# mmSir/SpatioTemporalEntropyModel

Hardware: AMD Instinct MI355X
Metric: frames/s (higher is better)
Workload: dtype f32; 1 GPU; configs[1]: SpatioTemporalPriorModel_Res(256,192) training step on mbt2018(192,192) latents, 16 septuplets x 7 frames x 256x256 per GPU, EMLoss, clip 1.0 + Adam 1e-4 / aux Adam 1e-3; per_gpu_batch=16, global_batch=16, parallelism=dp1, stream_priorities=latents=0,side=-1,compute=-1, stream_cu_masks=latents=block:160, plan_selectors=library defaults

## Files before the change

### include/stem_hip.h

```cpp
#ifndef STEM_HIP_H
#define STEM_HIP_H

#include <stddef.h>
#include <stdint.h>

#ifdef __cplusplus
extern "C" {
#endif

const char *stem_last_error(void);
int stem_abi_version(void);

void *stem_tape_create(void);
void stem_tape_destroy(void *tape);
int stem_tape_length(void *tape);
int stem_tape_add_call(void *tape, void *fn, int nargs, const unsigned char *kinds, const long long *ivals, const double *fvals,
                       const long long *ideltas);
int stem_tape_add_wait(void *tape, void *waiting_stream, void *signalling_stream);
int stem_tape_add_event(void *tape, void *event, void *stream, int wait);
int stem_tape_replay(void *tape, int lo, int hi, long long n);
int stem_tape_set_iarg(void *tape, int entry, int arg, long long value);
int stem_tape_set_farg(void *tape, int entry, int arg, double pattern);
int stem_tape_entry_recordable(void *fn);
int stem_copy_d2d(void *dst, const void *src, size_t nbytes, void *stream);
int stem_zero_bytes(void *dst, size_t nbytes, void *stream);
int stem_stream_flag_create(void **flag);
int stem_stream_flag_destroy(void *flag);
int stem_stream_flag_wait_ge(void *flag, unsigned value, void *stream);
int stem_stream_flag_write(void *flag, unsigned value, void *stream);
int stem_tuning_set(const char *name, int value);
int stem_tuning_get(const char *name);

enum {
    STEM_PACK_CONV_FWD = 0,
    STEM_PACK_CONV_DGRAD = 1,
    STEM_PACK_DECONV_FWD = 2,
    STEM_PACK_DECONV_DGRAD = 3,
    STEM_PACK_CONV_FWD_C4 = 4
};
int stem_pack_weight(const float *w, float *wp, int K, int C, int R, int S, int role, int masked, void *stream);
size_t stem_packed_weight_elems(int K, int C, int R, int S, int role);
enum { STEM_UNPACK_DECONV = 1, STEM_UNPACK_ACCUMULATE = 2 };
int stem_unpack_wgrad(const float *dwp, float *dw, int K, int C, int R, int S, int splits, int flags, void *stream);

typedef struct {
    const float *w;
    float *wp;
    int K, C, R, S, role, masked;
} stem_pack_desc;
typedef struct {
    const float *dwp;
    float *dw;
    int K, C, R, S, splits;
    int flags;
} stem_unpack_desc;
int stem_pack_weights_multi(const stem_pack_desc *descs, int n, void *stream);
int stem_unpack_wgrads_multi(const stem_unpack_desc *descs, int n, void *stream);
typedef struct {
    const float *part;
    float *db;
    int K, parts, accumulate, reserved;
} stem_bias_final_desc;
int stem_bias_grad_final_multi(const stem_bias_final_desc *descs, int n, void *stream);

enum { STEM_ACT_NONE = 0, STEM_ACT_LRELU = 1 };
// ... 287 lines not shown
```

### spatiotemporalentropymodel_amd/config.py

```python
from __future__ import annotations

import contextlib
import dataclasses
import os
from dataclasses import dataclass


@dataclass
class StemRuntimeConfig:
    analysis_f16x3: bool = True
    first_layer_f16x3: bool = True
    engine_f16x3: bool = True
    engine_strided_f16x3: bool = True
    engine_transposed_f16x3: bool = True
    engine_ctx_f16x3: bool = True
    engine_wgrad_f16x3: bool = True
    engine_records: bool = True
    layers_f16x3: bool = True
    layers_f16x3_maxpix: int = 1 << 30
    layers_wide_minpix: int = 32768
    trainer_overwrite_grads: bool = True
    adam_block_max: bool = True
    engine_overlap: bool = True
    engine_split_pack: bool = True
    engine_pack_pair: bool = True
    engine_branch: bool = True
    engine_tail_ordered: bool = True
    stream_prio: str = ""
    stream_cumask: str = ""
    dp_threaded: int = 3
    dp_min_bytes: int = 8 << 20
    dist_backend: str = ""
    dist_single: bool = False
    pin_ranks: bool = True
    ar_persistent: bool = True
    ar_stepwise: bool = False
    ar_force_batch: bool = False
    ar_concurrent: bool = True
    ar_no_batch: bool = False


_ENV = {
    "analysis_f16x3": "STEM_F16X3", "first_layer_f16x3": "STEM_C4GDN_F16X3", "engine_f16x3": "STEM_ENGINE_F16X3",
    "engine_strided_f16x3": "STEM_ENGINE_STRIDED_F16X3", "engine_transposed_f16x3": "STEM_ENGINE_TRANSPOSED_F16X3", "engine_ctx_f16x3": "STEM_ENGINE_CTX_F16X3",
    "engine_wgrad_f16x3": "STEM_ENGINE_WGRAD_F16X3", "engine_records": "STEM_ENGINE_RECORDS", "layers_f16x3": "STEM_LAYERS_F16X3",
    "layers_f16x3_maxpix": "STEM_LAYERS_F16X3_MAXPIX", "layers_wide_minpix": "STEM_LAYERS_WIDE_MINPIX",
    "adam_block_max": "STEM_ADAM_BLOCK_MAX", "trainer_overwrite_grads": "STEM_TRAINER_OVERWRITE_GRADS", "engine_overlap": "STEM_ENGINE_OVERLAP",
    "engine_split_pack": "STEM_ENGINE_SPLIT_PACK", "engine_pack_pair": "STEM_ENGINE_PACK_PAIR", "engine_branch": "STEM_ENGINE_BRANCH",
    "engine_tail_ordered": "STEM_ENGINE_TAIL_ORDERED",
    "stream_prio": "STEM_STREAM_PRIO", "stream_cumask": "STEM_STREAM_CUMASK", "dp_min_bytes": "STEM_DP_MIN_BYTES", "dp_threaded": "STEM_DP_THREADED",
    "dist_backend": "STEM_DIST_BACKEND", "dist_single": "STEM_DIST_SINGLE", "pin_ranks": "STEM_PIN_RANKS",
    "ar_persistent": "STEM_AR_PERSISTENT", "ar_stepwise": "STEM_AR_STEPWISE",
    "ar_force_batch": "STEM_AR_FORCE_BATCH", "ar_concurrent": "STEM_AR_CONCURRENT", "ar_no_batch": "STEM_AR_NO_BATCH",
}


def _parse(kind, text):
    if kind is bool:
        return text.strip() not in ("", "0", "false", "False", "no", "off")
    if kind is int:
        return int(text)
    return text


def from_env(environ=None) -> StemRuntimeConfig:
    environ = os.environ if environ is None else environ
    cfg = StemRuntimeConfig()
    for f in dataclasses.fields(cfg):
        name = _ENV[f.name]
        if name in environ:
            setattr(cfg, f.name, _parse(type(f.default), environ[name]))
    return cfg
# ... 48 lines not shown
```

### spatiotemporalentropymodel_amd/csrc/pack.hip

```cpp
#include <stdarg.h>

#include "stem_common.h"

static thread_local char g_err[512] = "";
void stem_set_error(const char *fmt, ...)
{
    va_list ap;
    va_start(ap, fmt);
    vsnprintf(g_err, sizeof(g_err), fmt, ap);
    va_end(ap);
}
STEM_EXPORT const char *stem_last_error(void) { return g_err; }
STEM_EXPORT int stem_abi_version(void) { return 5; }

static int g_tuning[STEM_TUNE_COUNT] = {0};
static const char *const kTuningNames[STEM_TUNE_COUNT] = {"fx3_tile", "fx3_split", "wg3_split", "arp_workers", "fx3_depth", "fx3_gen_tile", "fx3_mfma", "fx3_gen_mfma", "fx3_gen_img", "fx3_img_w", "wg3_row", "wg3_minch", "tconv_cps", "arp_giveup_at", "unpack_mb", "igemm_cfg", "igemm_fuse_cfg", "igemm_split", "wgrad_cfg"};
static int g_ran[STEM_RAN_COUNT] = {0};
static const char *const kRanNames[STEM_RAN_COUNT] = {"igemm_ran_cfg", "igemm_ran_split", "wgrad_ran_cfg", "fx3_ran_form", "fx3_ran_split", "fx3_ran_mfma", "wg3_ran_form", "wg3_ran_taps", "wg3_ran_split", "fx3_col_ran_tile", "fx3_col_ran_depth", "fx3_col_ran_mfma", "tconv_ran_tile", "tconv_ran_cps", "tconv_ran_split0", "tconv_ran_split1", "tconv_ran_split2", "tconv_ran_split3"};
void stem_ran_note(int id, int value) { g_ran[id] = value; }
int stem_tuning(int id) { return g_tuning[id]; }
STEM_EXPORT int stem_tuning_set(const char *name, int value)
{
    STEM_CHECK_ARG(name && value >= 0, "stem_tuning_set: null name or negative value");
    for (int i = 0; i < STEM_RAN_COUNT; ++i)
        STEM_CHECK_ARG(strcmp(name, kRanNames[i]), "stem_tuning_set: %s is get-only (the plan of the most recent launch)", name);
// ... 71 lines not shown
    const int n = d.Bd * d.T;
    for (int k = threadIdx.x; k < n; k += 256) {
        const int b = k / d.T, t = k - b * d.T;
        float v = d.w[a * d.sa + b * d.sb + t];
        if (d.masked & 3) {
            const int r = t / d.S, s = t - r * d.S;
            if (r > d.R / 2 || (r == d.R / 2 && s >= d.S / 2 + ((d.masked >> 2) & 1))) {
                v = 0.f;
                if ((d.masked & 3) == 2) d.w[a * d.sa + b * d.sb + t] = 0.f;
            }
        }
        tile[k] = v;
    }
    __syncthreads();
    for (int k = threadIdx.x; k < n; k += 256) {
        const int t = k / d.Bd, b = k - t * d.Bd;
        d.out[((size_t)t * d.A + a) * d.Bd + b] = tile[b * d.T + t];
    }
}

struct UnpackD {
    const float *dwp;
    float *dw;
    int A, Bd, T, splits, block0, accumulate, mb;
};
struct UnpackTable {
    UnpackD d[MAXD];
    int n;
};
constexpr int UNPACK_MB = 64, UNPACK_MB_MAX = 192;
__global__ __launch_bounds__(256) void unpack_multi_kernel(const UnpackTable tb)
{
    extern __shared__ float tile[];
    int i = 0;
    while (i + 1 < tb.n && (int)blockIdx.x >= tb.d[i + 1].block0) ++i;
    const UnpackD d = tb.d[i];
    const int mb = d.mb;
    const int chunks = (d.Bd + mb - 1) / mb;
    const int blk = blockIdx.x - d.block0;
    const int a = blk / chunks, b0 = (blk - a * chunks) * mb;
    const int nb = d.Bd - b0 < mb ? d.Bd - b0 : mb;
    const int n = nb * d.T;
    const size_t slab = (size_t)d.T * d.A * d.Bd;
    const bool vec = nb == mb && (d.Bd & 3) == 0 && ((reinterpret_cast<uintptr_t>(d.dwp) | reinterpret_cast<uintptr_t>(d.dw)) & 15) == 0 &&
                     ((size_t)d.Bd * d.T) % 4 == 0 && (slab & 3) == 0;
    if (vec) {
        const int q = mb / 4, n4 = d.T * q;
        for (int k = threadIdx.x; k < n4; k += 256) {
            const int t = k / q, b4 = k - t * q;
            const f32x4 *src = reinterpret_cast<const f32x4 *>(d.dwp + ((size_t)t * d.A + a) * d.Bd + b0) + b4;
            f32x4 v0 = {0.f, 0.f, 0.f, 0.f}, v1 = {0.f, 0.f, 0.f, 0.f};
            int sp = 0;
            for (; sp + 3 < d.splits; sp += 4) {
                const f32x4 x0 = src[(size_t)sp * (slab / 4)], x1 = src[(size_t)(sp + 1) * (slab / 4)];
                const f32x4 x2 = src[(size_t)(sp + 2) * (slab / 4)], x3 = src[(size_t)(sp + 3) * (slab / 4)];
                v0 += x0; v1 += x1; v0 += x2; v1 += x3;
            }
            for (; sp + 1 < d.splits; sp += 2) {
                const f32x4 x0 = src[(size_t)sp * (slab / 4)], x1 = src[(size_t)(sp + 1) * (slab / 4)];
                v0 += x0; v1 += x1;
            }
            if (sp < d.splits) v0 += src[(size_t)sp * (slab / 4)];
            const f32x4 v = v0 + v1;
#pragma unroll
            for (int j = 0; j < 4; ++j) tile[(b4 * 4 + j) * (d.T + 1) + t] = v[j];
        }
        __syncthreads();
        float *dst = d.dw + ((size_t)a * d.Bd + b0) * d.T;
        for (int k4 = threadIdx.x; k4 < n / 4; k4 += 256) {
            f32x4 v;
#pragma unroll
            for (int j = 0; j < 4; ++j) {
                const int k = 4 * k4 + j, b = k / d.T, t = k - b * d.T;
                v[j] = tile[b * (d.T + 1) + t];
            }
            f32x4 *o = reinterpret_cast<f32x4 *>(dst) + k4;
            *o = d.accumulate ? *o + v : v;
        }
        return;
    }
    for (int k = threadIdx.x; k < n; k += 256) {
        const int t = k / nb, b = k - t * nb;
        const float *src = d.dwp + ((size_t)t * d.A + a) * d.Bd + b0 + b;
        float v0 = 0.f, v1 = 0.f;
        int s = 0;
        for (; s + 1 < d.splits; s += 2) {
            v0 += src[s * slab];
            v1 += src[(s + 1) * slab];
        }
        if (s < d.splits) v0 += src[s * slab];
        tile[b * (d.T + 1) + t] = v0 + v1;
    }
    __syncthreads();
    float *dst = d.dw + ((size_t)a * d.Bd + b0) * d.T;
    for (int k = threadIdx.x; k < n; k += 256) {
        const int b = k / d.T, t = k - b * d.T;
        const float v = tile[b * (d.T + 1) + t];
        dst[k] = d.accumulate ? dst[k] + v : v;
    }
}

__global__ void pack_c4_kernel(const float *w, float *out, int K, int C, int T)
{
    const int i = blockIdx.x * blockDim.x + threadIdx.x;
    if (i >= K * 128) return;
    const int k = i >> 7, r = i & 127, t = r >> 2, c = r & 3;
    out[i] = (t < T && c < C) ? w[((size_t)k * C + c) * T + t] : 0.f;
}

constexpr int UNPACK_BT = 32;
__global__ __launch_bounds__(256) void unpack_kernel(const float *dwp, float *dw, int A, int Bd, int T, int splits, int accumulate)
{
    extern __shared__ float tile[];
    const int a = blockIdx.x, b0 = blockIdx.y * UNPACK_BT;
    const int nb = Bd - b0 < UNPACK_BT ? Bd - b0 : UNPACK_BT;
    const int n = nb * T;
    const size_t slab = (size_t)T * A * Bd;
    for (int i = threadIdx.x; i < n; i += 256) {
        const int t = i / nb, b = i - t * nb;
        const float *src = dwp + ((size_t)t * A + a) * Bd + b0 + b;
        float v0 = 0.f, v1 = 0.f;
        int s = 0;
// ... 146 lines not shown
            const stem_pack_desc &q = descs[base + i];
            PackD &d = tb.d[i];
            const int T = q.R * q.S;
            STEM_CHECK_ARG(q.w && q.wp && T >= 1 && T <= 25, "stem_pack_weights_multi: bad descriptor %d", base + i);
            STEM_CHECK_ARG(role_geometry(q.role, q.K, q.C, T, &d.A, &d.Bd, &d.sa, &d.sb) == 0,
                           "stem_pack_weights_multi: role %d not supported in the multi-tensor path", q.role);
            d.w = const_cast<float *>(q.w);
            d.out = q.wp;
            d.T = T; d.R = q.R; d.S = q.S; d.masked = q.masked;
            d.block0 = blocks;
            blocks += d.A;
            const size_t need = (size_t)d.Bd * T * sizeof(float);
            if (need > lds) lds = need;
        }
        STEM_CHECK_ARG(lds <= 160 * 1024, "stem_pack_weights_multi: slab of %zu B exceeds LDS", lds);
        if (lds > 64 * 1024)
            (void)hipFuncSetAttribute((const void *)pack_multi_kernel, hipFuncAttributeMaxDynamicSharedMemorySize, (int)lds);
        if (blocks) hipLaunchKernelGGL(pack_multi_kernel, dim3(blocks), dim3(256), lds, st, tb);
        STEM_LAUNCH_CHECK("pack_multi");
    }
    return 0;
}

STEM_EXPORT int stem_unpack_wgrads_multi(const stem_unpack_desc *descs, int n, void *stream)
{
    STEM_CHECK_ARG(descs && n >= 0, "stem_unpack_wgrads_multi: bad arguments");
    hipStream_t st = (hipStream_t)stream;
    for (int base = 0; base < n; base += MAXD) {
        UnpackTable tb;
        tb.n = n - base < MAXD ? n - base : MAXD;
        int blocks = 0;
        size_t lds = 0;
        for (int i = 0; i < tb.n; ++i) {
            const stem_unpack_desc &q = descs[base + i];
            UnpackD &d = tb.d[i];
            STEM_CHECK_ARG(q.dwp && q.dw && q.splits >= 1, "stem_unpack_wgrads_multi: bad descriptor %d", base + i);
            d.dwp = q.dwp; d.dw = q.dw;
            d.T = q.R * q.S;
            const int deconv = q.flags & STEM_UNPACK_DECONV;
            d.accumulate = (q.flags & STEM_UNPACK_ACCUMULATE) ? 1 : 0;
            d.A = deconv ? q.C : q.K;
            d.Bd = deconv ? q.K : q.C;
            d.splits = q.splits;
            d.block0 = blocks;
            const int forced_mb = stem_tuning(STEM_TUNE_UNPACK_MB);
            d.mb = UNPACK_MB;
            if (forced_mb) {
                d.mb = forced_mb;
            } else {
                for (int mb = UNPACK_MB_MAX; mb > UNPACK_MB; mb -= 32)
                    if (d.Bd % mb == 0 && (long)d.A * (d.Bd / mb) >= 512) {
                        d.mb = mb;
                        break;
                    }
            }
            blocks += d.A * cdiv(d.Bd, d.mb);
            const size_t need = (size_t)d.mb * (d.T + 1) * sizeof(float);
            if (need > lds) lds = need;
        }
        if (blocks) hipLaunchKernelGGL(unpack_multi_kernel, dim3(blocks), dim3(256), lds, st, tb);
        STEM_LAUNCH_CHECK("unpack_multi");
    }
    return 0;
}

STEM_EXPORT int stem_unpack_wgrad(const float *dwp, float *dw, int K, int C, int R, int S, int splits, int flags,
                                  void *stream)
{
    STEM_CHECK_ARG(dwp && dw && splits >= 1, "stem_unpack_wgrad: bad arguments");
    const int T = R * S;
    const int deconv = flags & STEM_UNPACK_DECONV;
    const int A = deconv ? C : K, Bd = deconv ? K : C;
    const size_t lds = (size_t)UNPACK_BT * (T + 1) * sizeof(float);
    STEM_CHECK_ARG(lds <= 64 * 1024, "stem_unpack_wgrad: %d taps exceed the staging tile", T);
    hipLaunchKernelGGL(unpack_kernel, dim3(A, cdiv(Bd, UNPACK_BT)), dim3(256), lds, (hipStream_t)stream, dwp, dw, A, Bd, T, splits,
                       (flags & STEM_UNPACK_ACCUMULATE) ? 1 : 0);
    STEM_LAUNCH_CHECK("unpack");
    return 0;
}

STEM_EXPORT int stem_nchw_to_nhwc(const float *x, float *y, int ldy, int B, int C, int H, int W, void *stream)
{
    STEM_CHECK_ARG(x && y && ldy >= C, "stem_nchw_to_nhwc: bad arguments");
    const int HW = H * W;
// ... 36 lines not shown
```

### spatiotemporalentropymodel_amd/engine.py

```python
from __future__ import annotations

import collections

import torch

from . import _lib
from . import config as _config
from . import functional as F
from . import layers as _layers

class _Switch:

    def __init__(self, field):
        self.field = field

    def __get__(self, obj, owner=None):
        return getattr(_config._RUNTIME or _config.runtime(), self.field)


class _Act:
    __slots__ = ("x", "p", "rec")

    def __init__(self, x, p=None, rec=None):
        self.x, self.p, self.rec = x, p, rec
# ... 130 lines not shown
        return _Act(F.deconv2d_fwd(a.x, self.wp_fwd, m.bias, self.K, self.R, self.R, self.stride, self.pad, self.opad, act, out=out))

    def fwd(self, x, act=F.ACT_NONE, out=None):
        return self.forward(_Act(x), act, out=out).x

    def input_grad(self, dy, xact=None, planes=False, x_shape=None):
        if self.tail_event is not None:
            self.eng._wait_tail(self)
        face = self.faces[1]
        epi = F.GEN_EPI_DACT if xact is not None else F.GEN_EPI_BIAS
        if face.kind == "gen":
            return _Act(*F.conv2d_f16x3_gen(dy.planes(), self.wp6_dgrad, None, self.C, self.R, self.R, self.stride, self.pad,
                                            epi=epi, z=xact, want_planes=planes))
        if face.kind == "phases":
            return _Act(*F.tconv2d_f16x3(dy.planes(), self.wp6_dgrad, None, self.C, self.R, epi=epi, z=xact, want_planes=planes,
                                         fine_hw=tuple(xact.shape[2:]) if xact is not None else None))
        x_shape = xact.shape if xact is not None else x_shape
        if self.kind == "conv":
            return _Act(F.conv2d_dgrad(dy.x, self.wp_dgrad, x_shape, self.K, self.R, self.R, self.stride, self.pad, xact=xact))
        return _Act(F.deconv2d_dgrad(dy.x, self.wp_dgrad, x_shape, self.K, self.R, self.R, self.stride, self.pad, self.opad, xact=xact))

    def reads_dy_planes(self, x):
        return self.faces[1].kind != "f32" if self.faces[1] is not None else (self.wg3 and x.p is not None)

    def weight_grad(self, x, dy):
        at_hand = (x.p is not None) + (dy.p is not None)
        if self.fx3t:
            fn, args = self._wgrad_t, ((x.planes(), dy.planes()) if self.kind == "conv" else (dy.planes(), x.planes())) + (dy.x,)
        elif self.wg3 and at_hand >= (2 if self.need_dgrad else 1):
            fn, args = self._wgrad3, (x.planes(record=False), dy.planes(record=False), dy.x)
        else:
            fn, args = self._wgrad, (x.x, dy.x)
        side = self.eng.side_stream(dy.x.device, self.lane)
        if side is None:
            return fn(*args)
        F.stream_wait(side, F.cur_stream(dy.x.device))
        with F.on_stream(side):
            fn(*args)
        for t in args:
            (t.data if isinstance(t, F.F16Planes) else t).record_stream(side)

    def _wgrad_t(self, fine_p, coarse_p, dy):
        conv = self.kind == "conv"
        Kk = self.K if conv else self.C
        key = ("fp16t",) + tuple(fine_p.shape)
        if key not in self._slabs:
# ... 334 lines not shown

    def _drop_tail(self):
        self.join_tail()
        self._tail_last = None
        self._tail_waited.clear()
        for l in self.layers:
            l.tail_event = None

    def unpack_all(self):
        for lane in sorted({l.lane for l in self.layers}):
            self._group_ready([l for l in self.layers if l.lane == lane], [])

    grad_ready_hook = None

    def _group_ready(self, layers, extra_params):
        dev = layers[0].mod.weight.device
        side = self.side_stream(dev, layers[0].lane)
        if side is None:
            return self._group_ready_on_stream(layers, extra_params)
        F.stream_wait(side, F.cur_stream(dev))
        with F.on_stream(side):
            self._group_ready_on_stream(layers, extra_params)

    def _group_ready_on_stream(self, layers, extra_params):
        bdescs = [l.pending_bias for l in layers if getattr(l, "pending_bias", None) is not None]
        for l in layers:
            l.pending_bias = None
        if bdescs:
            F.bias_grad_final_multi(bdescs)
        descs = [l.unpack_desc() for l in layers if l.pending is not None]
        if descs:
            arr = (_lib.UnpackDesc * len(descs))(*descs)
            F.unpack_wgrads_multi(arr)
        if self.grad_ready_hook is not None:
            params = [p for l in layers for p in (l.mod.weight, l.mod.bias) if p is not None] + list(extra_params)
            if params:
                hook = self.grad_ready_hook
                F.tape_py(lambda: hook(params))

    def join_side_stream(self):
        for st in self._side.values():
            F.stream_wait(F.cur_stream(st.device), st)

    def _wait_fwd32_packs(self):
        if self._fwd32_pack_event is not None:
            F.event_wait(F.cur_stream(), self._fwd32_pack_event)

    def _wait_dgrad_packs(self):
        if self._dgrad_pack_event is not None:
            F.event_wait(F.cur_stream(), self._dgrad_pack_event)
            self._dgrad_pack_event = None

    def forward(self, y_cur, y_cond, training: bool, rate_coef=None):
        self.ensure_packed()
        self._checked = True
        try:
# ... 89 lines not shown
            else:
                z_hat, lik_z = F.eb_forward(z, pack, medians=eb._medians_vec())
            acts["z_hat"], acts["hd0"], acts["hd2"], _ = self._chain_forward(self.HD, _Act(z_hat, rec=rec.get("z_hat")), out=epm_in[:, o_hp:o_hp + P], planes=ep)
        if not fused:
            target = F.sub(yc, yd) if self.residual else (yc if F.nhwc_ld(yc) == Cin else F.copy_channels(yc, F.empty_nhwc(B, Cin, H, W, dev)))
        if self.has_spm:
            if not fused:
                t_hat = F.add(target, gc._noise_like(target)) if training else F.round_(target)
                acts["t_hat"] = _Act(t_hat)
            if ctx_split_done is not None:
                F.event_wait(F.cur_stream(dev), ctx_split_done)
            self.CTX.forward(acts["t_hat"], out=epm_in[:, o_ctx:o_ctx + P])
        if bs is not None:
            F.stream_wait(main, bs)
        acts["epm_in"], acts["e0"], acts["e2"], gp = self._chain_forward(self.EPM, _Act(epm_in), planes=ep)
        gp = gp.x
        scales, means = gp[:, :Cin], gp[:, Cin:]
        if fused:
            dgp = F.empty_nhwc(B, 2 * Cin, H, W, dev)
            gc_out, lik_y, k["dlik_y"], part_y, k["qg"] = F.gc_forward_train(
                target, scales, means, rate_coef[0], scale_bound=gc._scale_bound, lik_bound=gc._lik_bound,
                backward=(dgp[:, :Cin], dgp[:, Cin:]), record=self.EPM[0].fx3 and self.use_records, **gc._noise_slot(target))
            k["dgp"] = dgp
            k["loss3"] = F.em_loss_finalize(part_y, part_z, rate_coef[1])
            if not self.has_spm:
                y_hat = gc_out
        else:
            noise = gc._noise_like(target) if training else None
            gc_out, lik_y = F.gc_forward(target, scales, means, noise=noise, scale_bound=gc._scale_bound, lik_bound=gc._lik_bound)
            if self.has_spm:
                y_hat = F.add(t_hat, yd if F.nhwc_ld(yd) == Cin else F.copy_channels(yd, F.empty_nhwc(B, Cin, H, W, dev))) if self.residual else t_hat
            else:
                y_hat = gc_out
        k.update(he_in=he_in, he0=acts["he0"].x, he2=acts["he2"].x, z_hat=z_hat, pack=pack, hd0=acts["hd0"].x, hd2=acts["hd2"].x,
                 epm_in=epm_in, tp0=tp0, tp2=tp2, yd=yd, t_hat=t_hat, e0=acts["e0"].x, e2=acts["e2"].x, gp=gp, gc_out=gc_out,
                 offs=(o_tp, o_hp, o_ctx), P=P, Cin=Cin)
        return y_hat, lik_y, lik_z, k

    def eval_rate(self, y_cur, y_cond, num_pixels, acc=None, weight=1.0):
        self.ensure_packed()
        self._checked = True
        try:
            return self._eval_rate(y_cur, y_cond, num_pixels, acc, weight)
        finally:
            self._checked = False

    def _eval_rate(self, y_cur, y_cond, num_pixels, acc, weight):
# ... 121 lines not shown
```

### spatiotemporalentropymodel_amd/functional.py

```python
from __future__ import annotations

import ctypes as C
import functools
import os

import torch

from . import _lib
from . import config as _config

PACK_CONV_FWD, PACK_CONV_DGRAD, PACK_DECONV_FWD, PACK_DECONV_DGRAD, PACK_CONV_FWD_C4 = 0, 1, 2, 3, 4
ACT_NONE, ACT_LRELU = 0, 1
CONV_MASKED_A = 0x100
LRELU_SLOPE = 0.01
EB_NPARAM = 58


def _stream():
    try:
        return torch._C._cuda_getCurrentRawStream(torch._C._cuda_getDevice())
    except AttributeError:
        return torch.cuda.current_stream().cuda_stream


# ... 1655 lines not shown
    B, Cc, H, W = sym.shape
    ldm = _pitch(means, "means", sym.shape) if means is not None else 0
    if chan_means is not None:
        _chan_vec(chan_means, Cc, "chan_means")
    y_hat = out if out is not None else empty_nhwc(B, Cc, H, W, sym.device)
    ldo = _pitch(y_hat, "out", sym.shape)
    _chk(_lib.hip().stem_symbols_unpack(sym.data_ptr(), _ptr(means), ldm, _ptr(chan_means), y_hat.data_ptr(), ldo, B, H, W, Cc, _stream()))
    return y_hat


SUMSQ_SCRATCH = 2048


def sumsq_accumulator(device):
    return torch.zeros(1 + SUMSQ_SCRATCH, dtype=torch.float64, device=device)


def sumsq(g, acc, overwrite=False):
    assert acc.numel() >= 1 + SUMSQ_SCRATCH
    fn = _lib.hip().stem_sumsq_set if overwrite else _lib.hip().stem_sumsq
    _chk(fn(g.data_ptr(), g.numel(), acc.data_ptr(), _stream()))


def clip_scale(g, sumsq_acc, max_norm):
    _chk(_lib.hip().stem_clip_scale(g.data_ptr(), g.numel(), sumsq_acc.data_ptr(), float(max_norm), _stream()))


def axpy_(y, x, a):
    _chk(_lib.hip().stem_axpy(y.data_ptr(), x.data_ptr(), float(a), y.numel(), _stream()))
    return y


def adam_step(p, g, m, v, sumsq_acc, max_norm, gscale, lr, beta1, beta2, eps, step, zero_grad=False):
    fn = _lib.hip().stem_adam_step_zero if zero_grad else _lib.hip().stem_adam_step
    _chk(fn(p.data_ptr(), g.data_ptr(), m.data_ptr(), v.data_ptr(), p.numel(), _ptr(sumsq_acc),
            max_norm, gscale, lr, beta1, beta2, eps, step, _stream()))


def adam_step_bmax(p, g, m, v, sumsq_acc, max_norm, gscale, lr, beta1, beta2, eps, step, bmax, zero_grad=False):
    _chk(_lib.hip().stem_adam_step_bmax(p.data_ptr(), g.data_ptr(), m.data_ptr(), v.data_ptr(), p.numel(), _ptr(sumsq_acc),
                                        max_norm, gscale, lr, beta1, beta2, eps, step, int(bool(zero_grad)), bmax.data_ptr(), _stream()))


def adam_ranges(ranges):
    flat = [int(c) for r in ranges for c in r]
    return (C.c_int * len(flat))(*flat)
# ... 268 lines not shown
```

### spatiotemporalentropymodel_amd/tape.py

```python
from __future__ import annotations

import ctypes as C
import struct
import warnings

import torch
from torch.utils._python_dispatch import TorchDispatchMode

from . import _lib
from . import functional as F


class TapeRefused(RuntimeError):
    """the schedule cannot be replayed faithfully (it is not static, or it contains device work a tape does not hold)"""


def _pattern(ty, value):
    if ty is C.c_float:
        return struct.unpack("<d", struct.pack("<fI", float(value), 0))[0]
    return float(value)


class LaunchTape:

# ... 292 lines not shown
        self._reset(None)

    def _reset(self, key):
        self.key, self.calls, self.tape, self.first = key, 0, None, None
        self.replays = 0
        self.refused = None

    taped = property(lambda self: self.tape is not None)

    def _counters(self):
        f = self.fused
        objs = [(f.opt, "t"), (f.aux_opt, "t"), (f.stem.entropy_bottleneck, "_noise_offset"), (f.stem.gaussian_conditional, "_noise_offset")]
        return [(o, a) for o, a in objs if hasattr(o, a)]

    def _refuse(self, why):
        self.refused, self.tape, self.first = str(why), None, None
        warnings.warn(f"TapedPFrameStep: running the ordinary schedule instead of a launch tape -- {why}", RuntimeWarning, stacklevel=3)

    def _key(self, y_cur, y_cond, num_pixels, grad_scale, reducer):
        f = self.fused
        clip = tuple(bool(o.max_norm is not None and o.max_norm > 0) for o in (f.opt, f.aux_opt))
        return (tuple(y_cur.shape), tuple(y_cond.shape), tuple(y_cur.stride()), tuple(y_cond.stride()), y_cur.dtype, y_cond.dtype, y_cur.device,
                int(num_pixels), float(grad_scale), id(reducer), F.cur_stream(y_cur.device).cuda_stream, clip, bool(f.clear_grad_in_adam),
                bool(f.adam_block_max), bool(f.overwrite_grads), bool(f.eng.tail_ordered))

    def step(self, y_cur, y_cond, num_pixels, grad_scale=1.0, reducer=None):
        key = self._key(y_cur, y_cond, num_pixels, grad_scale, reducer)
        if key != self.key:
            self._reset(key)
        f = self.fused
        if self.refused is not None:
            return f.step(y_cur, y_cond, num_pixels, grad_scale, reducer)
        if self.calls == 0:
            if f.opt._dev is not None or f.aux_opt._dev is not None:
                self._refuse("the optimiser keeps its step count / learning rate in device memory (enable_device_state)")
                return f.step(y_cur, y_cond, num_pixels, grad_scale, reducer)
            for name, t in (("y_cur", y_cur), ("y_cond", y_cond)):
                if F.nhwc_ld(t) is None and not t.is_contiguous():
                    self._refuse(f"{name} is neither NHWC nor contiguous: the schedule would convert it with a torch copy")
                    return f.step(y_cur, y_cond, num_pixels, grad_scale, reducer)
        self.calls += 1
        if self.calls <= self.WARMUP:
            return f.step(y_cur, y_cond, num_pixels, grad_scale, reducer)
        if self.calls == self.WARMUP + 1:
            self.in_cur = torch.empty_strided(y_cur.size(), y_cur.stride(), dtype=y_cur.dtype, device=y_cur.device)
            self.in_cond = torch.empty_strided(y_cond.size(), y_cond.stride(), dtype=y_cond.dtype, device=y_cond.device)
            if self.in_cur.stride() != y_cur.stride() or self.in_cond.stride() != y_cond.stride():
# ... 68 lines not shown
```

### spatiotemporalentropymodel_amd/trainer.py

```python
from __future__ import annotations

import contextlib
import math
import os

import torch

from . import config as _config
from . import functional as F
from .layers import join_wgrad_stream


SCHEDULE_DEFAULTS = {"STEM_STREAM_PRIO": "latents=0,side=-1,compute=-1", "STEM_STREAM_CUMASK": "latents=block:160"}


def tuned_schedule(device):
    for k, v in SCHEDULE_DEFAULTS.items():
        os.environ.setdefault(k, v)
    F.make_stream(device, "side")
    if "compute" in (F._STREAM_PRIO or {}):
        return torch.cuda.stream(F.make_stream(device, "compute"))
    return contextlib.nullcontext()


# ... 86 lines not shown
            raise ValueError("FusedPFrameStep needs the flat-buffer optimisers of optim.configure_optimizers(fused=True)")
        self._aux_loss = torch.zeros(1, dtype=torch.float32, device=eb.quantiles.device)
        self._grad_clean = False
        self.clear_grad_in_adam = True
        self.overwrite_grads = _config.runtime().trainer_overwrite_grads
        self.adam_block_max = _config.runtime().adam_block_max
        self._aux_stream = self.eng.side_stream(eb.quantiles.device) or F.make_stream(eb.quantiles.device, "side")
        self._aux_pending = False
        self._tail_plan = None
        self._done_event = torch.cuda.Event()

    def step(self, y_cur, y_cond, num_pixels, grad_scale=1.0, reducer=None):
        stem, opt, aux_opt, eng = self.stem, self.opt, self.aux_opt, self.eng
        eb = stem.entropy_bottleneck
        overwrite = bool(self.overwrite_grads)
        if overwrite or (self._grad_clean and opt._dev is None):
            for p in opt.flat.params:
                p.grad = p._flat_grad_view
        else:
            opt.flat.zero_grad()
        coef = -1.0 / (math.log(2.0) * num_pixels)
        y_hat, lik_y, lik_z, k = eng.forward(y_cur, y_cond, True, rate_coef=(coef, -1.0 / num_pixels))
        eng.accumulate_grads = not overwrite
        try:
            eng.backward(k, k["dlik_y"], k["dlik_z"])
        finally:
            eng.accumulate_grads = True
        if reducer is not None:
            F.tape_py(reducer.finish if hasattr(reducer, "finish") else reducer.all_reduce)
        join_wgrad_stream()
        main = F.cur_stream(y_hat.device)
        if self._aux_pending:
            F.stream_wait(main, self._aux_stream)
            self._aux_pending = False
        F.sumsq(opt.flat.grad, opt._sumsq, overwrite=True)
        clean = opt._dev is None and self.clear_grad_in_adam and not overwrite
        use_bmax = opt._dev is None and eng.use_fx3 and self.adam_block_max
        plan = None
        if (use_bmax and eng.tail_ordered and eng.pack_pair and eng.side_stream(main.device) is self._aux_stream
                and not torch.cuda.is_current_stream_capturing()):
            opt.ensure_block_maxima()
            plan = eng.tail_plan(opt)
        self._tail_plan = plan
        if plan is not None:
            opt.begin_ranges(grad_scale)
            eng.run_tail(plan, lambda table: opt.step_ranges(table, zero_grad=clean))
        else:
            opt.step(grad_scale=grad_scale, norm_is_current=True, zero_grad=clean, block_max=use_bmax)
        self._grad_clean = clean
        F.stream_wait(self._aux_stream, main)
        with F.on_stream(self._aux_stream):
            gn_copy = F.copy_d2d(torch.empty_like(opt._sumsq[:1]), opt._sumsq[:1])
            pack = F.eb_pack(eb._tensors14())
            F.eb_aux_loss_grad(eb.quantiles.detach(), pack, eb.target, eb.quantiles._flat_grad_view, loss_out=self._aux_loss)
            eb.quantiles.grad = eb.quantiles._flat_grad_view
            aux_opt.step()
            aux_copy = F.copy_d2d(torch.empty_like(self._aux_loss), self._aux_loss)
            done = self._done_event
# ... 308 lines not shown
```

Before: 10430 frames/s.

## Fold gradient-norm partial sums into per-group weight-gradient unpack launches

Each module group's weight-gradient unpack and bias finalisation now run in one kernel launch. That launch also writes per-workgroup float64 partial sums of squared gradients, and it covers the group's remaining parameter slices with sum-of-squares pieces. The trainer then reduces these partials instead of making a separate full pass over the flat gradient for clipping. The EM loss finalise is also moved to the side stream. This removes a full gradient read and some launches at the cost of more bookkeeping, coverage checks and a different summation order for the norm.

```diff
diff --git a/include/stem_hip.h b/include/stem_hip.h
--- a/include/stem_hip.h
+++ b/include/stem_hip.h
@@ -40,7 +40,8 @@
 };
 int stem_pack_weight(const float *w, float *wp, int K, int C, int R, int S, int role, int masked, void *stream);
 size_t stem_packed_weight_elems(int K, int C, int R, int S, int role);
-enum { STEM_UNPACK_DECONV = 1, STEM_UNPACK_ACCUMULATE = 2 };
+enum { STEM_UNPACK_DECONV = 1, STEM_UNPACK_ACCUMULATE = 2, STEM_UNPACK_BIAS = 4, STEM_UNPACK_SUMSQ = 8, STEM_UNPACK_PARTIALS = 16 };
+#define STEM_SUMSQ_PIECE 2048
 int stem_unpack_wgrad(const float *dwp, float *dw, int K, int C, int R, int S, int splits, int flags, void *stream);
 
 typedef struct {
diff --git a/spatiotemporalentropymodel_amd/config.py b/spatiotemporalentropymodel_amd/config.py
--- a/spatiotemporalentropymodel_amd/config.py
+++ b/spatiotemporalentropymodel_amd/config.py
@@ -26,6 +26,7 @@
     engine_pack_pair: bool = True
     engine_branch: bool = True
     engine_tail_ordered: bool = True
+    engine_fold_glue: bool = True
     stream_prio: str = ""
     stream_cumask: str = ""
     dp_threaded: int = 3
@@ -47,7 +48,7 @@
     "layers_f16x3_maxpix": "STEM_LAYERS_F16X3_MAXPIX", "layers_wide_minpix": "STEM_LAYERS_WIDE_MINPIX",
     "adam_block_max": "STEM_ADAM_BLOCK_MAX", "trainer_overwrite_grads": "STEM_TRAINER_OVERWRITE_GRADS", "engine_overlap": "STEM_ENGINE_OVERLAP",
     "engine_split_pack": "STEM_ENGINE_SPLIT_PACK", "engine_pack_pair": "STEM_ENGINE_PACK_PAIR", "engine_branch": "STEM_ENGINE_BRANCH",
-    "engine_tail_ordered": "STEM_ENGINE_TAIL_ORDERED",
+    "engine_tail_ordered": "STEM_ENGINE_TAIL_ORDERED", "engine_fold_glue": "STEM_ENGINE_FOLD_GLUE",
     "stream_prio": "STEM_STREAM_PRIO", "stream_cumask": "STEM_STREAM_CUMASK", "dp_min_bytes": "STEM_DP_MIN_BYTES", "dp_threaded": "STEM_DP_THREADED",
     "dist_backend": "STEM_DIST_BACKEND", "dist_single": "STEM_DIST_SINGLE", "pin_ranks": "STEM_PIN_RANKS",
     "ar_persistent": "STEM_AR_PERSISTENT", "ar_stepwise": "STEM_AR_STEPWISE",
diff --git a/spatiotemporalentropymodel_amd/csrc/norm_partial.h b/spatiotemporalentropymodel_amd/csrc/norm_partial.h
--- /dev/null
+++ b/spatiotemporalentropymodel_amd/csrc/norm_partial.h
@@ -0,0 +1,14 @@
+#pragma once
+#include "stem_common.h"
+
+constexpr int NORM_RED = 4;
+
+__device__ inline double block_sum_f64(double v, double *red)
+{
+#pragma unroll
+    for (int o = 32; o; o >>= 1) v += __shfl_down(v, o);
+    __syncthreads();
+    if ((threadIdx.x & 63) == 0) red[threadIdx.x >> 6] = v;
+    __syncthreads();
+    return ((red[0] + red[1]) + red[2]) + red[3];
+}
diff --git a/spatiotemporalentropymodel_amd/csrc/pack.hip b/spatiotemporalentropymodel_amd/csrc/pack.hip
--- a/spatiotemporalentropymodel_amd/csrc/pack.hip
+++ b/spatiotemporalentropymodel_amd/csrc/pack.hip
@@ -1,6 +1,7 @@
 #include <stdarg.h>
 
 #include "stem_common.h"
+#include "norm_partial.h"
 
 static thread_local char g_err[512] = "";
 void stem_set_error(const char *fmt, ...)
@@ -118,22 +119,19 @@
 struct UnpackD {
     const float *dwp;
     float *dw;
-    int A, Bd, T, splits, block0, accumulate, mb;
+    int A, Bd, T, splits, block0, accumulate, mb, kind;
 };
 struct UnpackTable {
     UnpackD d[MAXD];
     int n;
 };
 constexpr int UNPACK_MB = 64, UNPACK_MB_MAX = 192;
-__global__ __launch_bounds__(256) void unpack_multi_kernel(const UnpackTable tb)
-{
-    extern __shared__ float tile[];
-    int i = 0;
-    while (i + 1 < tb.n && (int)blockIdx.x >= tb.d[i + 1].block0) ++i;
-    const UnpackD d = tb.d[i];
+template <bool NORM>
+__device__ __forceinline__ double unpack_block(const UnpackD &d, const int blk, float *tile)
+{
+    double sq = 0.0;
     const int mb = d.mb;
     const int chunks = (d.Bd + mb - 1) / mb;
-    const int blk = blockIdx.x - d.block0;
     const int a = blk / chunks, b0 = (blk - a * chunks) * mb;
     const int nb = d.Bd - b0 < mb ? d.Bd - b0 : mb;
     const int n = nb * d.T;
@@ -171,9 +169,11 @@
                 v[j] = tile[b * (d.T + 1) + t];
             }
             f32x4 *o = reinterpret_cast<f32x4 *>(dst) + k4;
-            *o = d.accumulate ? *o + v : v;
-        }
-        return;
+            if (d.accumulate) v = *o + v;
+            *o = v;
+            if (NORM) sq += (double)v[0] * v[0] + (double)v[1] * v[1] + (double)v[2] * v[2] + (double)v[3] * v[3];
+        }
+        return sq;
     }
     for (int k = threadIdx.x; k < n; k += 256) {
         const int t = k / nb, b = k - t * nb;
@@ -191,9 +191,74 @@
     float *dst = d.dw + ((size_t)a * d.Bd + b0) * d.T;
     for (int k = threadIdx.x; k < n; k += 256) {
         const int b = k / d.T, t = k - b * d.T;
-        const float v = tile[b * (d.T + 1) + t];
-        dst[k] = d.accumulate ? dst[k] + v : v;
-    }
+        float v = tile[b * (d.T + 1) + t];
+        if (d.accumulate) v = dst[k] + v;
+        dst[k] = v;
+        if (NORM) sq += (double)v * v;
+    }
+    return sq;
+}
+__device__ __forceinline__ const UnpackD &unpack_desc_of(const UnpackTable &tb, const int block)
+{
+    int i = 0;
+    while (i + 1 < tb.n && block >= tb.d[i + 1].block0) ++i;
+    return tb.d[i];
+}
+__global__ __launch_bounds__(256) void unpack_multi_kernel(const UnpackTable tb)
+{
+    extern __shared__ float tile[];
+    const UnpackD d = unpack_desc_of(tb, blockIdx.x);
+    unpack_block<false>(d, blockIdx.x - d.block0, tile);
+}
+
+__device__ __forceinline__ double bias_final_block(const UnpackD &d, const int cb, float *red)
+{
+    const int lane = threadIdx.x & 63, w = threadIdx.x >> 6;
+    const int c = cb * 64 + lane, K = d.A, parts = d.splits;
+    float s[4] = {0.f, 0.f, 0.f, 0.f};
+    if (c < K)
+        for (int p0 = 4 * w; p0 < parts; p0 += 16) {
+#pragma unroll
+            for (int j = 0; j < 4; ++j)
+                if (p0 + j < parts) s[j] += d.dwp[(size_t)(p0 + j) * K + c];
+        }
+#pragma unroll
+    for (int j = 0; j < 4; ++j) red[(4 * w + j) * 64 + lane] = s[j];
+    __syncthreads();
+    double sq = 0.0;
+    if (w == 0 && c < K) {
+        float v = 0.f;
+#pragma unroll
+        for (int q = 0; q < 16; ++q) v += red[q * 64 + lane];
+        if (d.accumulate) v = d.dw[c] + v;
+        d.dw[c] = v;
+        sq = (double)v * v;
+    }
+    return sq;
+}
+__device__ __forceinline__ double sumsq_piece(const UnpackD &d, const int blk)
+{
+    const int e0 = blk * STEM_SUMSQ_PIECE, e1 = d.A - e0 < STEM_SUMSQ_PIECE ? d.A : e0 + STEM_SUMSQ_PIECE;
+    double sq = 0.0;
+    for (int e = e0 + threadIdx.x; e < e1; e += 256) sq += (double)d.dw[e] * d.dw[e];
+    return sq;
+}
+__global__ __launch_bounds__(256) void grad_group_finish_kernel(const UnpackTable tb, double *part)
+{
+    extern __shared__ __attribute__((aligned(16))) float smem[];
+    double *wsum = reinterpret_cast<double *>(smem);
+    float *tile = smem + 2 * NORM_RED;
+    const UnpackD d = unpack_desc_of(tb, blockIdx.x);
+    const int blk = blockIdx.x - d.block0;
+    double sq;
+    if (d.kind == STEM_UNPACK_BIAS)
+        sq = bias_final_block(d, blk, tile);
+    else if (d.kind == STEM_UNPACK_SUMSQ)
+        sq = sumsq_piece(d, blk);
+    else
+        sq = unpack_block<true>(d, blk, tile);
+    sq = block_sum_f64(sq, wsum);
+    if (threadIdx.x == 0) part[blockIdx.x] = sq;
 }
 
 __global__ void pack_c4_kernel(const float *w, float *out, int K, int C, int T)
@@ -386,44 +451,97 @@
     return 0;
 }
 
+namespace {
+void unpack_plan(const stem_unpack_desc &q, UnpackD &d, int &blocks, size_t &lds)
+{
+    d.dwp = q.dwp; d.dw = q.dw;
+    d.kind = 0;
+    d.T = q.R * q.S;
+    const int deconv = q.flags & STEM_UNPACK_DECONV;
+    d.accumulate = (q.flags & STEM_UNPACK_ACCUMULATE) ? 1 : 0;
+    d.A = deconv ? q.C : q.K;
+    d.Bd = deconv ? q.K : q.C;
+    d.splits = q.splits;
+    d.block0 = blocks;
+    const int forced_mb = stem_tuning(STEM_TUNE_UNPACK_MB);
+    d.mb = UNPACK_MB;
+    if (forced_mb) {
+        d.mb = forced_mb;
+    } else {
+        for (int mb = UNPACK_MB_MAX; mb > UNPACK_MB; mb -= 32)
+            if (d.Bd % mb == 0 && (long)d.A * (d.Bd / mb) >= 512) {
+                d.mb = mb;
+                break;
+            }
+    }
+    blocks += d.A * cdiv(d.Bd, d.mb);
+    const size_t need = (size_t)d.mb * (d.T + 1) * sizeof(float);
+    if (need > lds) lds = need;
+}
+bool finish_plan(const stem_unpack_desc &q, UnpackD &d, int &blocks, size_t &lds)
+{
+    memset(&d, 0, sizeof(d));
+    d.dwp = q.dwp; d.dw = q.dw;
+    d.block0 = blocks;
+    if (q.flags & STEM_UNPACK_BIAS) {
+        if (!q.dwp || !q.dw || q.K < 1 || q.splits < 1) return false;
+        d.kind = STEM_UNPACK_BIAS;
+        d.A = q.K; d.splits = q.splits;
+        d.accumulate = (q.flags & STEM_UNPACK_ACCUMULATE) ? 1 : 0;
+        blocks += cdiv(q.K, 64);
+        if (lds < 16 * 64 * sizeof(float)) lds = 16 * 64 * sizeof(float);
+    } else {
+        if (!q.dw || q.K < 0) return false;
+        d.kind = STEM_UNPACK_SUMSQ;
+        d.A = q.K;
+        blocks += cdiv(q.K, STEM_SUMSQ_PIECE);
+    }
+    return true;
+}
+}
+
 STEM_EXPORT int stem_unpack_wgrads_multi(const stem_unpack_desc *descs, int n, void *stream)
 {
     STEM_CHECK_ARG(descs && n >= 0, "stem_unpack_wgrads_multi: bad arguments");
     hipStream_t st = (hipStream_t)stream;
-    for (int base = 0; base < n; base += MAXD) {
-        UnpackTable tb;
-        tb.n = n - base < MAXD ? n - base : MAXD;
-        int blocks = 0;
-        size_t lds = 0;
-        for (int i = 0; i < tb.n; ++i) {
-            const stem_unpack_desc &q = descs[base + i];
-            UnpackD &d = tb.d[i];
-            STEM_CHECK_ARG(q.dwp && q.dw && q.splits >= 1, "stem_unpack_wgrads_multi: bad descriptor %d", base + i);
-            d.dwp = q.dwp; d.dw = q.dw;
-            d.T = q.R * q.S;
-            const int deconv = q.flags & STEM_UNPACK_DECONV;
-            d.accumulate = (q.flags & STEM_UNPACK_ACCUMULATE) ? 1 : 0;
-            d.A = deconv ? q.C : q.K;
-            d.Bd = deconv ? q.K : q.C;
-            d.splits = q.splits;
-            d.block0 = blocks;
-            const int forced_mb = stem_tuning(STEM_TUNE_UNPACK_MB);
-            d.mb = UNPACK_MB;
-            if (forced_mb) {
-                d.mb = forced_mb;
-            } else {
-                for (int mb = UNPACK_MB_MAX; mb > UNPACK_MB; mb -= 32)
-                    if (d.Bd % mb == 0 && (long)d.A * (d.Bd / mb) >= 512) {
-                        d.mb = mb;
-                        break;
-                    }
-            }
-            blocks += d.A * cdiv(d.Bd, d.mb);
-            const size_t need = (size_t)d.mb * (d.T + 1) * sizeof(float);
-            if (need > lds) lds = need;
-        }
-        if (blocks) hipLaunchKernelGGL(unpack_multi_kernel, dim3(blocks), dim3(256), lds, st, tb);
-        STEM_LAUNCH_CHECK("unpack_multi");
+    const stem_unpack_desc *slots = nullptr;
+    for (int i = 0; i < n; ++i)
+        if (descs[i].flags & STEM_UNPACK_PARTIALS) {
+            STEM_CHECK_ARG(!slots && descs[i].dw && descs[i].K >= 0 && descs[i].C >= 0,
+                           "stem_unpack_wgrads_multi: descriptor %d: one STEM_UNPACK_PARTIALS descriptor with its buffer, first slot and slot count", i);
+            slots = &descs[i];
+        }
+    for (int pass = slots ? 0 : 1; pass < 2; ++pass) {
+        long total = 0;
+        for (int base = 0; base < n;) {
+            UnpackTable tb;
+            tb.n = 0;
+            int blocks = 0;
+            size_t lds = 0;
+            for (; base < n && tb.n < MAXD; ++base) {
+                const stem_unpack_desc &q = descs[base];
+                if (q.flags & STEM_UNPACK_PARTIALS) continue;
+                UnpackD &d = tb.d[tb.n++];
+                if (q.flags & (STEM_UNPACK_BIAS | STEM_UNPACK_SUMSQ)) {
+                    STEM_CHECK_ARG(slots && finish_plan(q, d, blocks, lds), "stem_unpack_wgrads_multi: bad descriptor %d (a bias or sum-of-squares "
+                                   "descriptor needs a STEM_UNPACK_PARTIALS descriptor in the call)", base);
+                    continue;
+                }
+                STEM_CHECK_ARG(q.dwp && q.dw && q.splits >= 1, "stem_unpack_wgrads_multi: bad descriptor %d", base);
+                unpack_plan(q, d, blocks, lds);
+            }
+            if (pass && blocks && !slots) hipLaunchKernelGGL(unpack_multi_kernel, dim3(blocks), dim3(256), lds, st, tb);
+            if (pass && blocks && slots) {
+                lds += NORM_RED * sizeof(double);
+                STEM_CHECK_ARG(lds <= 64 * 1024, "stem_unpack_wgrads_multi: tile of %zu B exceeds LDS", lds);
+                hipLaunchKernelGGL(grad_group_finish_kernel, dim3(blocks), dim3(256), lds, st, tb,
+                                   reinterpret_cast<double *>(slots->dw) + slots->K + total);
+            }
+            if (pass) STEM_LAUNCH_CHECK("unpack_multi");
+            total += blocks;
+        }
+        STEM_CHECK_ARG(pass || total == slots->C, "stem_unpack_wgrads_multi: %ld workgroups where the caller expects %d partial-sum slots", total,
+                       slots->C);
     }
     return 0;
 }
diff --git a/spatiotemporalentropymodel_amd/engine.py b/spatiotemporalentropymodel_amd/engine.py
--- a/spatiotemporalentropymodel_amd/engine.py
+++ b/spatiotemporalentropymodel_amd/engine.py
@@ -176,6 +176,9 @@
 
     def reads_dy_planes(self, x):
         return self.faces[1].kind != "f32" if self.faces[1] is not None else (self.wg3 and x.p is not None)
+
+    def bias_deferred(self):
+        return self.mod.bias is not None and not (self.fx3t and self.kind == "deconv")
 
     def weight_grad(self, x, dy):
         at_hand = (x.p is not None) + (dy.p is not None)
@@ -556,16 +559,105 @@
         with F.on_stream(side):
             self._group_ready_on_stream(layers, extra_params)
 
+    fold_glue = _Switch("engine_fold_glue")
+
+    _NormGroup = collections.namedtuple("_NormGroup", "finish rest rest_descs slot0 nslots")
+    _NormPlan = collections.namedtuple("_NormPlan", "groups part nslots flat")
+
+    def _norm_groups(self):
+        eb = self.m.entropy_bottleneck
+        groups = [(self.EPM, []), ([self.CTX] if self.has_spm else [], []), (self.TPM if self.has_tpm else [], []),
+                  (self.HD, eb._tensors14()), (self.HE, [])]
+        return [g for g in groups if g[0]]
+
+    def norm_plan(self, flat, slots=None):
+        cache = getattr(self, "_norm_cache", None)
+        if cache is not None and cache[0] is flat:
+            return cache[1]
+        plan = self._build_norm_plan(flat, slots or F.grad_group_finish_slots)
+        if slots is None:
+            self._norm_cache = (flat, plan)
+        return plan
+
+    def _build_norm_plan(self, flat, slots):
+        where = {id(p): (off, p.numel()) for p, off in zip(flat.params, flat.offsets)}
+        groups, cover, slot = {}, [], 0
+        for layers, extra in self._norm_groups():
+            finish, rest, descs = [], [], []
+            for l in layers:
+                for p, deferred in ((l.mod.weight, True), (l.mod.bias, l.bias_deferred())):
+                    if p is None:
+                        continue
+                    if id(p) not in where:
+                        return None
+                    (finish if deferred else rest).append(where[id(p)])
+                descs.append(_lib.UnpackDesc(0, 0, l.K, l.C, l.R, l.R, 1, F.UNPACK_DECONV if l.kind == "deconv" else 0))
+                if l.mod.bias is not None and l.bias_deferred():
+                    descs.append(_lib.UnpackDesc(0, 0, l.K, 0, 0, 0, 1, F.UNPACK_BIAS))
+            for p in extra:
+                if id(p) not in where:
+                    return None
+                rest.append(where[id(p)])
+            rest += [(off + n, -n % 4) for off, n in finish + rest if n % 4]
+            merged = []
+            for off, n in sorted(rest):
+                if merged and merged[-1][0] + merged[-1][1] == off:
+                    merged[-1] = (merged[-1][0], merged[-1][1] + n)
+                else:
+                    merged.append((off, n))
+            rest_descs = [F.sumsq_desc(flat.grad, off, n) for off, n in merged]
+            nslots = slots(descs + rest_descs)
+            groups[id(layers[0])] = self._NormGroup(tuple(sorted(finish)), tuple(merged), rest_descs, slot, nslots)
+            slot += nslots
+            cover += finish + merged
+        end = 0
+        for off, n in sorted(cover):
+            if off != end:
+                return None
+            end = off + n
+        if end != flat.numel:
+            return None
+        part = torch.zeros(slot, dtype=torch.float64, device=flat.grad.device) if flat.grad.is_cuda else None
+        return self._NormPlan(groups, part, slot, flat)
+
+    def begin_norm(self, flat):
+        self._norm, self._norm_done = None, set()
+        if self.fold_glue and self.grad_ready_hook is None:
+            self._norm = self.norm_plan(flat)
+        return self._norm
+
+    def end_norm(self, complete=True):
+        plan, self._norm = self._norm, None
+        if plan is not None and complete and self._norm_done != set(plan.groups):
+            raise RuntimeError("StemEngine: a module group's gradients did not pass through _group_ready in this backward: the "
+                               "partial sums of the gradient norm are incomplete")
+        return plan
+
+    _norm = None
+
+    def _group_finish_norm(self, plan, layers, descs, bdescs):
+        g = plan.groups.get(id(layers[0]))
+        base = plan.flat.grad.data_ptr()
+        got = sorted([(d.dw - base) // 4 for d in descs] + [(d.db - base) // 4 for d in bdescs])
+        if g is None or got != [off for off, _ in g.finish]:
+            raise RuntimeError("StemEngine: the gradients a finishing launch stores are not the ones the norm plan gives it")
+        n = F.grad_group_finish(descs + [F.bias_final_as_unpack(b) for b in bdescs] + g.rest_descs, plan.part, g.slot0)
+        if n != g.nslots:
+            raise RuntimeError(f"StemEngine: a finishing launch of {n} workgroups where the norm plan holds {g.nslots} slots")
+        self._norm_done.add(id(layers[0]))
+
     def _group_ready_on_stream(self, layers, extra_params):
         bdescs = [l.pending_bias for l in layers if getattr(l, "pending_bias", None) is not None]
         for l in layers:
             l.pending_bias = None
-        if bdescs:
-            F.bias_grad_final_multi(bdescs)
         descs = [l.unpack_desc() for l in layers if l.pending is not None]
-        if descs:
-            arr = (_lib.UnpackDesc * len(descs))(*descs)
-            F.unpack_wgrads_multi(arr)
+        if self._norm is not None:
+            self._group_finish_norm(self._norm, layers, descs, bdescs)
+        else:
+            if bdescs:
+                F.bias_grad_final_multi(bdescs)
+            if descs:
+                F.unpack_wgrads_multi((_lib.UnpackDesc * len(descs))(*descs))
         if self.grad_ready_hook is not None:
             params = [p for l in layers for p in (l.mod.weight, l.mod.bias) if p is not None] + list(extra_params)
             if params:
@@ -701,7 +793,17 @@
                 target, scales, means, rate_coef[0], scale_bound=gc._scale_bound, lik_bound=gc._lik_bound,
                 backward=(dgp[:, :Cin], dgp[:, Cin:]), record=self.EPM[0].fx3 and self.use_records, **gc._noise_slot(target))
             k["dgp"] = dgp
-            k["loss3"] = F.em_loss_finalize(part_y, part_z, rate_coef[1])
+            side = self.side_stream(dev) if self.fold_glue and self.grad_ready_hook is None else None
+            if side is not None:
+                cur = F.cur_stream(dev)
+                F.stream_wait(side, cur)
+                with F.on_stream(side):
+                    k["loss3"] = F.em_loss_finalize(part_y, part_z, rate_coef[1])
+                for t in (part_y, part_z):
+                    t.record_stream(side)
+                k["loss3"].record_stream(cur)
+            else:
+                k["loss3"] = F.em_loss_finalize(part_y, part_z, rate_coef[1])
             if not self.has_spm:
                 y_hat = gc_out
         else:
diff --git a/spatiotemporalentropymodel_amd/functional.py b/spatiotemporalentropymodel_amd/functional.py
--- a/spatiotemporalentropymodel_amd/functional.py
+++ b/spatiotemporalentropymodel_amd/functional.py
@@ -1701,6 +1701,55 @@
     _chk(fn(g.data_ptr(), g.numel(), acc.data_ptr(), _stream()))
 
 
+UNPACK_BIAS, UNPACK_SUMSQ, UNPACK_PARTIALS = 4, 8, 16
+SUMSQ_PIECE = _lib.header_macro("stem_hip.h", "STEM_SUMSQ_PIECE")
+
+
+def unpack_run_length(A, Bd):
+    forced = _lib.hip().stem_tuning_get(b"unpack_mb")
+    if forced:
+        return forced
+    for mb in range(192, 64, -32):
+        if Bd % mb == 0 and A * (Bd // mb) >= 512:
+            return mb
+    return 64
+
+
+def grad_group_finish_slots(descs):
+    n = 0
+    for d in descs:
+        if d.flags & UNPACK_BIAS:
+            n += (d.K + 63) // 64
+        elif d.flags & UNPACK_SUMSQ:
+            n += (d.K + SUMSQ_PIECE - 1) // SUMSQ_PIECE
+        else:
+            A, Bd = (d.C, d.K) if d.flags & UNPACK_DECONV else (d.K, d.C)
+            n += A * -(-Bd // unpack_run_length(A, Bd))
+    return n
+
+
+def bias_final_as_unpack(b):
+    return _lib.UnpackDesc(b.part, b.db, b.K, 0, 0, 0, b.parts, UNPACK_BIAS | (UNPACK_ACCUMULATE if b.accumulate else 0))
+
+
+def sumsq_desc(g, offset, count):
+    assert 0 <= offset and 0 <= count and offset + count <= g.numel()
+    return _lib.UnpackDesc(0, g.data_ptr() + 4 * offset, count, 0, 0, 0, 0, UNPACK_SUMSQ)
+
+
+def grad_group_finish(descs, part, slot0):
+    n = grad_group_finish_slots(descs)
+    assert part.dtype == torch.float64 and 0 <= slot0 and slot0 + n <= part.numel(), "grad_group_finish: partial-sum buffer too small"
+    arr = (_lib.UnpackDesc * (len(descs) + 1))(*descs, _lib.UnpackDesc(0, part.data_ptr(), slot0, n, 0, 0, 0, UNPACK_PARTIALS))
+    _chk(_lib.hip().stem_unpack_wgrads_multi(arr, len(arr), _stream()))
+    return n
+
+
+def sumsq_from_partials(part, nparts, acc):
+    assert part.dtype == torch.float64 and acc.dtype == torch.float64 and 0 <= nparts <= part.numel() and acc.numel() >= 3
+    _chk(_lib.hip().stem_em_loss_finalize(part.data_ptr(), nparts, None, 0, 1.0, acc.data_ptr(), _stream()))
+
+
 def clip_scale(g, sumsq_acc, max_norm):
     _chk(_lib.hip().stem_clip_scale(g.data_ptr(), g.numel(), sumsq_acc.data_ptr(), float(max_norm), _stream()))
 
diff --git a/spatiotemporalentropymodel_amd/tape.py b/spatiotemporalentropymodel_amd/tape.py
--- a/spatiotemporalentropymodel_amd/tape.py
+++ b/spatiotemporalentropymodel_amd/tape.py
@@ -338,7 +338,7 @@
         clip = tuple(bool(o.max_norm is not None and o.max_norm > 0) for o in (f.opt, f.aux_opt))
         return (tuple(y_cur.shape), tuple(y_cond.shape), tuple(y_cur.stride()), tuple(y_cond.stride()), y_cur.dtype, y_cond.dtype, y_cur.device,
                 int(num_pixels), float(grad_scale), id(reducer), F.cur_stream(y_cur.device).cuda_stream, clip, bool(f.clear_grad_in_adam),
-                bool(f.adam_block_max), bool(f.overwrite_grads), bool(f.eng.tail_ordered))
+                bool(f.adam_block_max), bool(f.overwrite_grads), bool(f.eng.tail_ordered), bool(f.eng.fold_glue))
 
     def step(self, y_cur, y_cond, num_pixels, grad_scale=1.0, reducer=None):
         key = self._key(y_cur, y_cond, num_pixels, grad_scale, reducer)
diff --git a/spatiotemporalentropymodel_amd/trainer.py b/spatiotemporalentropymodel_amd/trainer.py
--- a/spatiotemporalentropymodel_amd/trainer.py
+++ b/spatiotemporalentropymodel_amd/trainer.py
@@ -132,10 +132,16 @@
         coef = -1.0 / (math.log(2.0) * num_pixels)
         y_hat, lik_y, lik_z, k = eng.forward(y_cur, y_cond, True, rate_coef=(coef, -1.0 / num_pixels))
         eng.accumulate_grads = not overwrite
+        norm = eng.begin_norm(opt.flat) if reducer is None else None
         try:
             eng.backward(k, k["dlik_y"], k["dlik_z"])
+        except BaseException:
+            eng.end_norm(complete=False)
+            raise
         finally:
             eng.accumulate_grads = True
+        if norm is not None:
+            eng.end_norm()
         if reducer is not None:
             F.tape_py(reducer.finish if hasattr(reducer, "finish") else reducer.all_reduce)
         join_wgrad_stream()
@@ -143,7 +149,10 @@
         if self._aux_pending:
             F.stream_wait(main, self._aux_stream)
             self._aux_pending = False
-        F.sumsq(opt.flat.grad, opt._sumsq, overwrite=True)
+        if norm is not None:
+            F.sumsq_from_partials(norm.part, norm.nslots, opt._sumsq)
+        else:
+            F.sumsq(opt.flat.grad, opt._sumsq, overwrite=True)
         clean = opt._dev is None and self.clear_grad_in_adam and not overwrite
         use_bmax = opt._dev is None and eng.use_fx3 and self.adam_block_max
         plan = None
```

After: 10410 frames/s, median of 2. About the same (-0.2%).
